# MAPieschl/PointCloudProcessing

Measured on AMD Instinct MI355X. Metric: points/sec PointNet fwd+bwd N=1024 B=32 at 1/2/4/8 MI355X vs CPU ref, higher is better.
Workload: dtype bf16; 1 GPU; PointNet-cls training step (fwd + losses + bwd + grad all-reduce + Adam), N=1024 points, batch 32 per GPU, profile classification_pretrain, 23 classes / 12 parts, random-init weights; global_batch=32, points_per_cloud=1024, parallelism=dp1, launch=hipgraph

## Files before the change

### pointcloudprocessing_amd/csrc/pn_gemm.hip

```cpp
#include <vector>
#include "pn_common.h"
#include "pn_dense_wgrad.h"
#include "pn_gemm_core.h"
#include "pn_internal.h"
#include "pn_slab_reduce.h"

namespace pn {

template <int BM, int BN, int NS, bool B2>
__global__ __launch_bounds__(256) void wgrad_batch_kernel(const WgradBatch wb) {
  __shared__ __attribute__((aligned(16))) unsigned char lds_raw[GemmLds<BM, BN, NS>::BYTES];
  wgrad_batch_tile<BM, BN, NS, B2>(wb, (int)blockIdx.x, lds_raw);
}

template <int BM, int BN, int NS, bool B2>
__global__ __launch_bounds__(256) void wgrad_batch_dense_kernel(const WgradBatch wb, int n_w, const DenseWgradBatch db) {
  __shared__ __attribute__((aligned(16))) unsigned char lds_raw[GemmLds<BM, BN, NS>::BYTES];
  static_assert(GemmLds<BM, BN, NS>::BYTES >= 16 * 32 * 4, "the dense riders' LDS tile fits");
  if ((int)blockIdx.x >= n_w) {
    dense_wgrad_batch_body(db, (int)blockIdx.x - n_w, reinterpret_cast<float(*)[32]>(lds_raw));
    return;
  }
  wgrad_batch_tile<BM, BN, NS, B2>(wb, (int)blockIdx.x, lds_raw);
}

struct WgLds {
  static constexpr int PITCH = Geo<64>::PITCH;
  static constexpr int W = 2 * 128 * PITCH, A = W + 64 * PITCH, RED_BYTES = (A + 128 * PITCH) * 2, BYTES = RED_BYTES + 4 * 64 * 4;
  static_assert(BYTES <= 65536, "the fused weight-gradient tile's LDS exceeds the static __shared__ limit");
};
template <int BM, int BN, int NS, int MODE, bool A2, int EPI, bool ADD, bool MASK, bool AH, bool S16, bool W16 = false, bool WG = false>
__device__ __forceinline__ void rows_tile_t(const GemmArgs& g, const int bx, const int by, unsigned char* lds_raw, const WgArgs* wa = nullptr) {
  constexpr int BK = (NS == 3) ? 32 : 64;
  constexpr int PITCH = Geo<BK>::PITCH;
  constexpr int MT = BM / 64, NT = BN / 64;
  constexpr int WTM = BM / 2, WTN = BN / 2;
  constexpr int TILE_A = BM * PITCH, TILE_B = BN * PITCH;
  static_assert(!WG || (BM == 128 && BN == 64 && NS == 1 && MODE == MODE_BWD && EPI == EPI_STORE && AH && S16), "the fused weight-gradient tile");
  __bf16* Ahi = reinterpret_cast<__bf16*>(lds_raw);
  __bf16* Bhi = Ahi + (WG ? WgLds::W : TILE_A);
  __bf16* Alo = (NS == 3) ? (Bhi + TILE_B) : Ahi;
  __bf16* Blo = (NS == 3) ? (Alo + TILE_A) : Bhi;

  const int tid = threadIdx.x, lane = tid & 63, wave = tid >> 6;
  const int wm = wave >> 1, wn = wave & 1;
  const int wrow0 = wm * WTM, wcol0 = wn * WTN;

  f32x16 acc[MT][NT];
#pragma unroll
  for (int m = 0; m < MT; ++m)
#pragma unroll
    for (int n = 0; n < NT; ++n)
#pragma unroll
      for (int e = 0; e < 16; ++e) acc[m][n][e] = 0.f;

  const int cloud = bx / g.tiles_per_cloud, tin = bx - cloud * g.tiles_per_cloud;

  const int row_in_cloud0 = tin * BM;
  const int nrows = min(BM, g.N - row_in_cloud0);
  const long long row0 = (long long)cloud * g.N + row_in_cloud0;
  const int col0 = by * BN;
  const long long wbase = (long long)cloud * g.w_cloud_stride;
  pn_operand wop;
  wop.s1 = g.w; wop.s2 = nullptr; wop.ca = nullptr; wop.cb = nullptr; wop.cc = nullptr;
  wop.lo = -INFINITY; wop.h16 = 0;
  wop.ld = (MODE == MODE_FWD) ? g.C : g.K;

  NatStage<BM, BK, A2, AH> sa;
  TrnStage<BN, BK, false, false> sbT;
  NatStage<BN, BK, false, false> sbN;
  CopyStage<BN, BK> sbC;
  auto issue_chunk = [&](int k0) {
    if (!(g.dbg & 4)) sa.issue(g.a, row0 * g.a.ld, nrows, k0, tid);
    if constexpr (W16) {
      sbC.issue(g.w16, (long long)col0 * g.K, g.K, g.C - col0, k0, tid);
    } else if (MODE == MODE_FWD) {
      if (!(g.dbg & 8)) sbT.issue(wop, wbase + (long long)k0 * g.C + col0, BK, g.C - col0, tid);
    } else {
      sbN.issue(wop, wbase + (long long)col0 * g.K, g.C - col0, k0, tid);
    }
  };
  NatStage<BM, BK, false, true> swg;
  if constexpr (WG) swg.issue(wa->a, row0 * wa->a.ld, nrows, 0, tid);
  if (g.K > 0) issue_chunk(0);
  for (int k0 = 0; k0 < g.K; k0 += BK) {
    sa.pin();
    if constexpr (WG) {
      Ahi = reinterpret_cast<__bf16*>(lds_raw) + (k0 / BK) * TILE_A;
      Alo = Ahi;
    }
    sa.template finish<NS>(Ahi, Alo, g.a, nrows, k0, tid);
    if constexpr (W16) {
      sbC.pin();
      sbC.finish(Bhi, g.C - col0, tid);
    } else if (MODE == MODE_FWD) {
      sbT.pin();
      sbT.template finish<NS>(Bhi, Blo, wop, BK, g.C - col0, 0, tid);
    } else {
      sbN.pin();
      sbN.template finish<NS>(Bhi, Blo, wop, g.C - col0, k0, tid);
    }
    __syncthreads();
    if (k0 + BK < g.K) issue_chunk(k0 + BK);
    mma_chunk<MT, NT, BK, NS>(acc, Ahi, Alo, Bhi, Blo, wrow0, wcol0, lane);
    __syncthreads();
  }
  if constexpr (WG) {
    swg.pin();
    swg.template finish<1>(reinterpret_cast<__bf16*>(lds_raw) + WgLds::A, reinterpret_cast<__bf16*>(lds_raw) + WgLds::A, wa->a, nrows, 0, tid);
  }

  const int r = lane & 31, h = lane >> 5;
  const bool full = (nrows == BM) && (col0 + BN <= g.C);
  float* red = reinterpret_cast<float*>(lds_raw + (WG ? WgLds::RED_BYTES : 0));

  if (EPI == EPI_STORE) {
    float s1[NT], s2[NT];
#pragma unroll
    for (int n = 0; n < NT; ++n) {
      const int jl = wcol0 + n * 32 + r, j = col0 + jl;
      const bool jv = j < g.C;
      float bias = 0.f, msc = 0.f, msh = 0.f;
      if (jv && g.cloud_bias) bias = g.cloud_bias[(long long)cloud * g.cloud_bias_stride + j];
      if (jv && g.zmask) { msc = g.msc[j]; msh = g.msh[j]; }
      float a1 = 0.f, a2 = 0.f;
#pragma unroll
      for (int m = 0; m < MT; ++m) {
        const int il0 = wrow0 + m * 32 + 4 * h;
        if (full) {
          if (g.out && !(g.dbg & 1)) epi_store_block<true, ADD, MASK, true, S16>(acc[m][n], g, row0, il0, nrows, j, jv, bias, msc, msh, a1, a2);
          else epi_store_block<true, ADD, MASK, false, S16>(acc[m][n], g, row0, il0, nrows, j, jv, bias, msc, msh, a1, a2);
        } else {
          if (g.out) epi_store_block<false, ADD, MASK, true, S16>(acc[m][n], g, row0, il0, nrows, j, jv, bias, msc, msh, a1, a2);
          else epi_store_block<false, ADD, MASK, false, S16>(acc[m][n], g, row0, il0, nrows, j, jv, bias, msc, msh, a1, a2);
        }
      }
      s1[n] = a1 + __shfl_xor(a1, 32, 64);
      s2[n] = a2 + __shfl_xor(a2, 32, 64);
    }
    if (g.stat_partials && !(g.dbg & 2)) {
      if (h == 0) {
#pragma unroll
        for (int n = 0; n < NT; ++n) {
          const int jl = wcol0 + n * 32 + r;
          red[(wm * 2 + 0) * BN + jl] = s1[n];
          red[(wm * 2 + 1) * BN + jl] = s2[n];
        }
      }
      __syncthreads();
      if (tid < BN && col0 + tid < g.C) {
        float* p = g.stat_partials + (long long)bx * 2 * g.C + col0 + tid;
        p[0] = red[0 * BN + tid] + red[2 * BN + tid];
        p[g.C] = red[1 * BN + tid] + red[3 * BN + tid];
      }
    }
    if constexpr (WG) {
      __syncthreads();
      const __bf16* img = reinterpret_cast<const __bf16*>(lds_raw);
// ... 67 lines not shown
  __shared__ __attribute__((aligned(16))) unsigned char lds_raw[LDS_BYTES];
  if constexpr (MODE == MODE_WGRAD) {
    wgrad_tile<BM, BN, NS, A2, B2>(g, blockIdx.x, blockIdx.y, blockIdx.z, lds_raw);
  } else {
    int bx = blockIdx.x, by = 0;
    const int ncol = g.ncol;
    if (ncol > 1) {
      const int lin = blockIdx.x, nrow = (int)gridDim.x / ncol, full = (nrow / 8) * 8 * ncol;
      if (lin < full) {
        const int grp = lin / (8 * ncol), r = lin - grp * 8 * ncol;
        by = r >> 3;
        bx = grp * 8 + (r & 7);
      } else {
        const int l2 = lin - full, rem = nrow - (nrow / 8) * 8;
        bx = (nrow / 8) * 8 + l2 % rem;
        by = l2 / rem;
      }
    }
    if (g.a.h16) {
      if constexpr (NS == 1 && EPI == EPI_STORE) {
        if (g.w16) {
          if (g.store16) rows_tile_t<BM, BN, NS, MODE, A2, EPI, ADD, MASK, true, true, true>(g, bx, by, lds_raw);
          else rows_tile_t<BM, BN, NS, MODE, A2, EPI, ADD, MASK, true, false, true>(g, bx, by, lds_raw);
          return;
        }
      }
      if (EPI == EPI_STORE && g.store16) rows_tile_t<BM, BN, NS, MODE, A2, EPI, ADD, MASK, true, EPI == EPI_STORE>(g, bx, by, lds_raw);
      else rows_tile_t<BM, BN, NS, MODE, A2, EPI, ADD, MASK, true, false>(g, bx, by, lds_raw);
    } else {
      if (EPI == EPI_STORE && g.store16) rows_tile_t<BM, BN, NS, MODE, A2, EPI, ADD, MASK, false, EPI == EPI_STORE>(g, bx, by, lds_raw);
      else rows_tile_t<BM, BN, NS, MODE, A2, EPI, ADD, MASK, false, false>(g, bx, by, lds_raw);
    }
  }
}

template <bool ADD, bool MASK>
__global__ __launch_bounds__(256) void gemm_bwd_wgrad_kernel(const GemmArgs g, const WgArgs wa) {
  __shared__ __attribute__((aligned(16))) unsigned char lds_raw[WgLds::BYTES];
  if (g.w16) rows_tile_t<128, 64, 1, MODE_BWD, true, EPI_STORE, ADD, MASK, true, true, true, true>(g, (int)blockIdx.x, 0, lds_raw, &wa);
  else rows_tile_t<128, 64, 1, MODE_BWD, true, EPI_STORE, ADD, MASK, true, true, false, true>(g, (int)blockIdx.x, 0, lds_raw, &wa);
}

template <bool AH, bool S16>
__global__ __launch_bounds__(256) void gemm_bwd_reduce_kernel(const GemmArgs g, int n_gemm, const float* __restrict__ slabs, int per_group,
                                                              long long elems, float* __restrict__ red_out, int nb_per_group) {
  constexpr int LDS_BYTES = (128 + 64) * Geo<64>::PITCH * 2;
  static_assert(LDS_BYTES >= 8 * 32 * 4, "the riders' LDS tile fits");
  __shared__ __attribute__((aligned(16))) unsigned char lds_raw[LDS_BYTES];
  if ((int)blockIdx.x >= n_gemm) {
    const int bx = (int)blockIdx.x - n_gemm;
    slab_reduce_block(slabs, per_group, elems, red_out, bx % nb_per_group, bx / nb_per_group, reinterpret_cast<float(*)[32]>(lds_raw));
    return;
  }
  rows_tile_t<128, 64, 1, MODE_BWD, false, EPI_STORE, false, false, AH, S16>(g, (int)blockIdx.x, 0, lds_raw);
}

template <int BM, int BN, int NS, int MODE, bool A2, bool B2, int EPI, bool ADD = false, bool MASK = false>
static int launch(const GemmArgs& g, dim3 grid, hipStream_t st) {
  hipLaunchKernelGGL((gemm_kernel<BM, BN, NS, MODE, A2, B2, EPI, ADD, MASK>), grid, dim3(256), 0, st, g);
  PN_CHECK_LAUNCH();
  return PN_OK;
}

static bool aligned16(const void* p) { return (reinterpret_cast<uintptr_t>(p) & 15) == 0; }

static int check_operand(const pn_operand* o, const char* name) {
  PN_CHECK_ARG(o && o->s1, "%s: null operand", name);
  PN_CHECK_ARG(aligned16(o->s1) && (!o->s2 || aligned16(o->s2)), "%s: s1/s2 must be 16-byte aligned", name);
  PN_CHECK_ARG((!o->ca || aligned16(o->ca)) && (!o->cb || aligned16(o->cb)) && (!o->cc || aligned16(o->cc)),
               "%s: coefficient vectors must be 16-byte aligned", name);
  PN_CHECK_ARG(o->ld > 0 && o->ld % 4 == 0, "%s: ld must be a positive multiple of 4", name);
  PN_CHECK_ARG(o->h16 == 0 || (o->h16 == 1 && o->ld % 8 == 0), "%s: h16 must be 0 or 1, and 16-bit rows need ld %% 8 == 0", name);
  return PN_OK;
}

template <int MODE, bool A2, int EPI, bool ADD = false, bool MASK = false>
static int dispatch_rows(const GemmArgs& g_in, int prec, hipStream_t st) {
  GemmArgs g = g_in;
  const bool wide = g.C % 128 == 0;
  if (EPI == EPI_MAX) {
    g.ncol = cdiv(g.C, 128);
    dim3 grid(g.B * g.tiles_per_cloud * g.ncol);
    if (prec == PN_PREC_BF16X3) return launch<128, 128, 3, MODE, A2, false, EPI>(g, grid, st);
    return launch<128, 128, 1, MODE, A2, false, EPI>(g, grid, st);
  }
  const bool few = (long long)g.B * g.tiles_per_cloud * (g.C / 128) < 64;
  if (wide && !few) {
    g.ncol = g.C / 128;
    dim3 grid(g.B * g.tiles_per_cloud * g.ncol);
    if (prec == PN_PREC_BF16X3) return launch<128, 128, 3, MODE, A2, false, EPI, ADD, MASK>(g, grid, st);
    return launch<128, 128, 1, MODE, A2, false, EPI, ADD, MASK>(g, grid, st);
  }
  g.ncol = cdiv(g.C, 64);
  dim3 grid(g.B * g.tiles_per_cloud * g.ncol);
  if (prec == PN_PREC_BF16X3) return launch<128, 64, 3, MODE, A2, false, EPI, ADD, MASK>(g, grid, st);
  return launch<128, 64, 1, MODE, A2, false, EPI, ADD, MASK>(g, grid, st);
}

template <bool A2>
static int dispatch_bwd(const GemmArgs& g, int prec, hipStream_t st) {
  const bool ha = g.addend != nullptr, hm = g.zmask != nullptr;
  if (ha && hm) return dispatch_rows<MODE_BWD, A2, EPI_STORE, true, true>(g, prec, st);
  if (ha) return dispatch_rows<MODE_BWD, A2, EPI_STORE, true, false>(g, prec, st);
  if (hm) return dispatch_rows<MODE_BWD, A2, EPI_STORE, false, true>(g, prec, st);
  return dispatch_rows<MODE_BWD, A2, EPI_STORE, false, false>(g, prec, st);
}

int conv_fwd(const pn_operand* x, const float* w, long long wcs, int B, int N, int K, int C, const float* cloud_bias,
             float* z, float* stat_partials, int prec, hipStream_t st, const void* w16) {
  PN_TRY(check_operand(x, "pn_conv_fwd.x"));
  PN_CHECK_ARG(!x->s2, "pn_conv_fwd: the forward operand has no second source");
  PN_CHECK_ARG(B > 0 && N > 0, "pn_conv_fwd: B and N must be positive (B=%d N=%d)", B, N);
  PN_CHECK_ARG(K >= 64 && K % 64 == 0, "pn_conv_fwd: K must be a multiple of 64 (K=%d)", K);
  PN_CHECK_ARG(C >= 64 && C % 64 == 0, "pn_conv_fwd: C must be a multiple of 64 (C=%d)", C);
  PN_CHECK_ARG(x->ld >= K, "pn_conv_fwd: x.ld < K");
  PN_CHECK_ARG(w && aligned16(w), "pn_conv_fwd: w null or unaligned");
  const int store16 = (prec & PN_STORE_BF16) ? 1 : 0;
  prec &= ~PN_STORE_BF16;
  PN_CHECK_ARG(prec == PN_PREC_BF16 || prec == PN_PREC_BF16X3, "pn_conv_fwd: bad prec %d", prec);
  GemmArgs g;
  memset(&g, 0, sizeof(g));
  g.store16 = store16;
  g.a = *x; g.w = w; g.w_cloud_stride = wcs; g.B = B; g.N = N; g.K = K; g.C = C;
  g.tiles_per_cloud = cdiv(N, 128);
  g.out = z; g.cloud_bias = cloud_bias; g.cloud_bias_stride = C; g.stat_partials = stat_partials;
  if (w16 && wcs == 0 && prec == PN_PREC_BF16 && x->h16 && (reinterpret_cast<uintptr_t>(w16) & 15) == 0 && K % 8 == 0)
    g.w16 = reinterpret_cast<const unsigned short*>(w16);
  static const int dbg = getenv("PN_GEMM_DBG") ? atoi(getenv("PN_GEMM_DBG")) : 0;
  g.dbg = dbg;
  return dispatch_rows<MODE_FWD, false, EPI_STORE>(g, prec, st);
}

int conv_fwd_max(const pn_operand* x, const float* w, int B, int N, int K, int C, const float* sgn, float* pmax, int* pidx,
                 float* stat_partials, int prec, hipStream_t st) {
  PN_TRY(check_operand(x, "pn_conv_fwd_max.x"));
  PN_CHECK_ARG(!x->s2, "pn_conv_fwd_max: the forward operand has no second source");
  PN_CHECK_ARG(B > 0 && N > 0, "pn_conv_fwd_max: B and N must be positive");
  PN_CHECK_ARG(K >= 64 && K % 64 == 0, "pn_conv_fwd_max: K must be a multiple of 64 (K=%d)", K);
  PN_CHECK_ARG(C >= 128 && C % 128 == 0, "pn_conv_fwd_max: C must be a multiple of 128 (C=%d)", C);
  PN_CHECK_ARG(x->ld >= K, "pn_conv_fwd_max: x.ld < K");
  PN_CHECK_ARG(w && aligned16(w) && sgn && pmax && pidx, "pn_conv_fwd_max: null pointer");
  PN_CHECK_ARG(prec == PN_PREC_BF16 || prec == PN_PREC_BF16X3, "pn_conv_fwd_max: bad prec %d", prec);
  GemmArgs g;
  memset(&g, 0, sizeof(g));
  g.a = *x; g.w = w; g.B = B; g.N = N; g.K = K; g.C = C;
  g.tiles_per_cloud = cdiv(N, 128);
  g.sgn = sgn; g.pmax = pmax; g.pidx = pidx; g.stat_partials = stat_partials;
  return dispatch_rows<MODE_FWD, false, EPI_MAX>(g, prec, st);
}

int conv_bwd_data(const pn_operand* dz, const float* w, long long wcs, int B, int N, int K, int C, const float* addend,
                  const float* zmask, const float* msc, const float* msh, float* out, float* stat_partials, int prec,
                  hipStream_t st, const void* w16, const float* col_bias, const WgradFuse* wf) {
  PN_TRY(check_operand(dz, "pn_conv_bwd_data.dz"));
  PN_CHECK_ARG(B > 0 && N > 0, "pn_conv_bwd_data: B and N must be positive");
  PN_CHECK_ARG(K >= 64 && K % 64 == 0, "pn_conv_bwd_data: K must be a multiple of 64 (K=%d)", K);
  PN_CHECK_ARG(C >= 64 && C % 64 == 0, "pn_conv_bwd_data: C must be a multiple of 64 (C=%d)", C);
  PN_CHECK_ARG(dz->ld >= K, "pn_conv_bwd_data: dz.ld < K");
  PN_CHECK_ARG(w && aligned16(w), "pn_conv_bwd_data: w null or unaligned");
  PN_CHECK_ARG(!zmask || (msc && msh), "pn_conv_bwd_data: zmask needs msc and msh");
  const int store16 = (prec & PN_STORE_BF16) ? 1 : 0;
  prec &= ~PN_STORE_BF16;
  PN_CHECK_ARG(prec == PN_PREC_BF16 || prec == PN_PREC_BF16X3, "pn_conv_bwd_data: bad prec %d", prec);
  GemmArgs g;
  memset(&g, 0, sizeof(g));
  g.store16 = store16;
  g.a = *dz; g.w = w; g.w_cloud_stride = wcs; g.B = B; g.N = N; g.K = K; g.C = C;
  g.tiles_per_cloud = cdiv(N, 128);
  g.out = out; g.addend = addend; g.zmask = zmask; g.msc = msc; g.msh = msh; g.stat_partials = stat_partials;
  g.cloud_bias = col_bias; g.cloud_bias_stride = 0;
  if (w16 && wcs == 0 && prec == PN_PREC_BF16 && dz->h16 && (reinterpret_cast<uintptr_t>(w16) & 15) == 0 && K % 8 == 0)
    g.w16 = reinterpret_cast<const unsigned short*>(w16);
  if (wf) {
    PN_TRY(check_operand(&wf->a, "pn_conv_bwd_data_wgrad.a"));
    PN_CHECK_ARG(prec == PN_PREC_BF16 && store16 && dz->h16 && dz->s2, "pn_conv_bwd_data_wgrad: bf16 operands, bf16 storage and a two-source dz");
    PN_CHECK_ARG(C == 64 && (K == 64 || K == 128), "pn_conv_bwd_data_wgrad: C must be 64 and K 64 or 128 (C=%d K=%d)", C, K);
    PN_CHECK_ARG(wf->Ci == C && wf->a.h16 && !wf->a.s2 && wf->a.ld >= wf->Ci, "pn_conv_bwd_data_wgrad: operand a must be a 64-channel bf16 single-source operand");
    PN_CHECK_ARG(wf->slab_rows == 64 || wf->slab_rows == 128, "pn_conv_bwd_data_wgrad: slab_rows must be 64 or 128 (%d)", wf->slab_rows);
    PN_CHECK_ARG(wf->slabs != nullptr, "pn_conv_bwd_data_wgrad: null slabs");
    const WgArgs wa{wf->a, wf->slabs, wf->slab_rows};
    g.ncol = 1;
    const dim3 grid(B * g.tiles_per_cloud);
    const bool ha = addend != nullptr, hm = zmask != nullptr;
    if (ha && hm) hipLaunchKernelGGL((gemm_bwd_wgrad_kernel<true, true>), grid, dim3(256), 0, st, g, wa);
    else if (ha) hipLaunchKernelGGL((gemm_bwd_wgrad_kernel<true, false>), grid, dim3(256), 0, st, g, wa);
    else if (hm) hipLaunchKernelGGL((gemm_bwd_wgrad_kernel<false, true>), grid, dim3(256), 0, st, g, wa);
    else hipLaunchKernelGGL((gemm_bwd_wgrad_kernel<false, false>), grid, dim3(256), 0, st, g, wa);
    PN_CHECK_LAUNCH();
    return PN_OK;
  }
  if (dz->s2) return dispatch_bwd<true>(g, prec, st);
  return dispatch_bwd<false>(g, prec, st);
}

int conv_bwd_data_reduce(const pn_operand* dz, const float* w, long long wcs, int B, int N, int K, int C, float* out, int prec, hipStream_t st,
                         const float* slabs, int n_slabs, int per_group, long long elems, float* red_out, bool* rode) {
  *rode = false;
  PN_TRY(check_operand(dz, "pn_conv_bwd_data.dz"));
  PN_CHECK_ARG(B > 0 && N > 0 && w && aligned16(w) && out && dz->ld >= K, "conv_bwd_data_reduce: bad arguments");
  PN_CHECK_ARG(slabs && red_out && n_slabs > 0 && per_group > 0 && n_slabs % per_group == 0 && elems > 0, "conv_bwd_data_reduce: bad sizes");
  const int store16 = (prec & PN_STORE_BF16) ? 1 : 0;
  prec &= ~PN_STORE_BF16;
  const long long nb = cdivll(elems, 32), riders = nb * (n_slabs / per_group), n_gemm = (long long)B * cdiv(N, 128);
  if (prec != PN_PREC_BF16 || dz->s2 || C != 64 || K < 64 || K % 64 != 0 || (dz->h16 != 0) != (store16 != 0) || n_gemm + riders >= (1ll << 30))
    return PN_OK;
  GemmArgs g;
  memset(&g, 0, sizeof(g));
  g.store16 = store16;
  g.a = *dz; g.w = w; g.w_cloud_stride = wcs; g.B = B; g.N = N; g.K = K; g.C = C;
  g.tiles_per_cloud = cdiv(N, 128);
  g.out = out; g.ncol = 1;
  const dim3 grid((unsigned)(n_gemm + riders));
  if (store16)
    hipLaunchKernelGGL((gemm_bwd_reduce_kernel<true, true>), grid, dim3(256), 0, st, g, (int)n_gemm, slabs, per_group, elems, red_out, (int)nb);
  else
    hipLaunchKernelGGL((gemm_bwd_reduce_kernel<false, false>), grid, dim3(256), 0, st, g, (int)n_gemm, slabs, per_group, elems, red_out, (int)nb);
  PN_CHECK_LAUNCH();
  *rode = true;
  return PN_OK;
}

template <int BM, int BN>
static int dispatch_wgrad(const GemmArgs& g, bool b2, int prec, dim3 grid, hipStream_t st) {
  if (prec == PN_PREC_BF16X3) {
    if (b2) return launch<BM, BN, 3, MODE_WGRAD, false, true, EPI_SLAB>(g, grid, st);
// ... 108 lines not shown
```

### pointcloudprocessing_amd/csrc/pn_gemm_core.h

```cpp
#pragma once
#include "pn_common.h"
#include "pn_internal.h"

namespace pn {

typedef __attribute__((ext_vector_type(8))) __bf16 bf16x8;
typedef __attribute__((ext_vector_type(16))) float f32x16;

enum { MODE_FWD = 0, MODE_BWD = 1, MODE_WGRAD = 2 };
enum { EPI_STORE = 0, EPI_MAX = 1, EPI_SLAB = 2 };

struct GemmArgs {
  pn_operand a;
  pn_operand b;
  const float* w;
  const unsigned short* w16;
  long long w_cloud_stride;
  int B, N;
  int K;
  int C;
  int Ci;
  int tiles_per_cloud;
  float* out;
  const float* cloud_bias;
  long long cloud_bias_stride;
  const float* addend;
  const float* zmask;
  const float* msc;
  const float* msh;
  float* stat_partials;
  const float* sgn;
  float* pmax;
  int* pidx;
  int store16;
  int ncol;
  int colsum;
  int dbg;
};
struct WgArgs {
  pn_operand a;
  float* slabs;
  int rows;
};

template <int BK>
struct Geo {
  static constexpr int PITCH = BK + 8;
};

__device__ __forceinline__ void cvt_store8(__bf16* hi, __bf16* lo, const float (&v)[8], bool split) {
  bf16x8 h;
#pragma unroll
  for (int e = 0; e < 8; ++e) h[e] = (__bf16)v[e];
  *reinterpret_cast<bf16x8*>(hi) = h;
  if (split) {
    bf16x8 l;
#pragma unroll
    for (int e = 0; e < 8; ++e) l[e] = (__bf16)(v[e] - (float)h[e]);
    *reinterpret_cast<bf16x8*>(lo) = l;
  }
}


template <int TR, int BK, bool HAS2, bool H16>
struct NatStage {
  static constexpr int CH = BK / 8;
  static constexpr int RP = 256 / CH;
  static constexpr int P = TR / RP;
  static constexpr int Q = H16 ? 1 : 2;
  float4 x[P][Q];
  float4 y[HAS2 ? P : 1][Q];

  __device__ __forceinline__ void issue(const pn_operand& op, long long base, int nvalid_rows, int k0, int tid) {
    const int ch = tid % CH, rin = tid / CH;
    const int k = k0 + ch * 8;
#pragma unroll
    for (int p = 0; p < P; ++p) {
      const int r = p * RP + rin;
      const long long rr = (r < nvalid_rows) ? r : (nvalid_rows - 1);
      if constexpr (H16) {
        x[p][0] = __builtin_bit_cast(float4, act_load8_raw(op.s1, base + rr * op.ld + k));
        if (HAS2) y[p][0] = __builtin_bit_cast(float4, act_load8_raw(op.s2, base + rr * op.ld + k));
      } else {
        const float* s = op.s1 + base + rr * op.ld + k;
        x[p][0] = *reinterpret_cast<const float4*>(s);
        x[p][1] = *reinterpret_cast<const float4*>(s + 4);
        if (HAS2) {
          const float* s2 = op.s2 + base + rr * op.ld + k;
          y[p][0] = *reinterpret_cast<const float4*>(s2);
          y[p][1] = *reinterpret_cast<const float4*>(s2 + 4);
        }
      }
    }
  }
  __device__ __forceinline__ void pin() {
#pragma unroll
    for (int p = 0; p < P; ++p)
#pragma unroll
      for (int q = 0; q < Q; ++q) {
        asm volatile("" : "+v"(x[p][q].x), "+v"(x[p][q].y), "+v"(x[p][q].z), "+v"(x[p][q].w));
        if (HAS2) asm volatile("" : "+v"(y[p][q].x), "+v"(y[p][q].y), "+v"(y[p][q].z), "+v"(y[p][q].w));
      }
  }
  template <int NS>
  __device__ __forceinline__ void finish(__bf16* __restrict__ Thi, __bf16* __restrict__ Tlo, const pn_operand& op,
                                         int nvalid_rows, int k0, int tid) {
    constexpr int PITCH = Geo<BK>::PITCH;
    const int ch = tid % CH, rin = tid / CH;
    const int k = k0 + ch * 8;
    float ca[8], cb[8], cc[8];
#pragma unroll
    for (int e = 0; e < 8; ++e) { ca[e] = 1.f; cb[e] = 0.f; cc[e] = 0.f; }
    if (op.ca) {
      const float4 t0 = *reinterpret_cast<const float4*>(op.ca + k), t1 = *reinterpret_cast<const float4*>(op.ca + k + 4);
      ca[0] = t0.x; ca[1] = t0.y; ca[2] = t0.z; ca[3] = t0.w; ca[4] = t1.x; ca[5] = t1.y; ca[6] = t1.z; ca[7] = t1.w;
    }
    if (HAS2 && op.cb) {
      const float4 t0 = *reinterpret_cast<const float4*>(op.cb + k), t1 = *reinterpret_cast<const float4*>(op.cb + k + 4);
      cb[0] = t0.x; cb[1] = t0.y; cb[2] = t0.z; cb[3] = t0.w; cb[4] = t1.x; cb[5] = t1.y; cb[6] = t1.z; cb[7] = t1.w;
    }
    if (op.cc) {
      const float4 t0 = *reinterpret_cast<const float4*>(op.cc + k), t1 = *reinterpret_cast<const float4*>(op.cc + k + 4);
      cc[0] = t0.x; cc[1] = t0.y; cc[2] = t0.z; cc[3] = t0.w; cc[4] = t1.x; cc[5] = t1.y; cc[6] = t1.z; cc[7] = t1.w;
    }
    const float lo = op.lo;
#pragma unroll
    for (int p = 0; p < P; ++p) {
      const int r = p * RP + rin;
      const bool rv = r < nvalid_rows;
      float v[8], w[8];
      if constexpr (H16) {
        bf16x8_unpack(__builtin_bit_cast(uint4, x[p][0]), v);
        if (HAS2) bf16x8_unpack(__builtin_bit_cast(uint4, y[p][0]), w);
      } else {
        v[0] = x[p][0].x; v[1] = x[p][0].y; v[2] = x[p][0].z; v[3] = x[p][0].w;
        v[4] = x[p][Q - 1].x; v[5] = x[p][Q - 1].y; v[6] = x[p][Q - 1].z; v[7] = x[p][Q - 1].w;
        if (HAS2) {
          w[0] = y[p][0].x; w[1] = y[p][0].y; w[2] = y[p][0].z; w[3] = y[p][0].w;
          w[4] = y[p][Q - 1].x; w[5] = y[p][Q - 1].y; w[6] = y[p][Q - 1].z; w[7] = y[p][Q - 1].w;
        }
      }
#pragma unroll
      for (int e = 0; e < 8; ++e) {
        float t = fmaf(ca[e], v[e], cc[e]);
        if (HAS2) t = fmaf(cb[e], w[e], t);
        v[e] = rv ? clamp_lo(t, lo) : 0.f;
      }
      cvt_store8(Thi + r * PITCH + ch * 8, Tlo + r * PITCH + ch * 8, v, NS == 3);
    }
  }
};

template <int TR, int BK, bool HAS2, bool H16>
struct TrnStage {
  static constexpr int KG = BK / 8;
  static constexpr int TRL = H16 ? TR / 2 : TR;
  static constexpr int TPG = 256 / TRL;
  static constexpr int P = (KG + TPG - 1) / TPG;
  static_assert(KG % TPG == 0 || TPG % KG == 0, "tile geometry");
  float x[P][8];
  float y[HAS2 ? P : 1][8];

  __device__ __forceinline__ void issue(const pn_operand& op, long long base, int nvalid_k, int nvalid_r, int tid) {
    const int rl = tid % TRL, kgin = tid / TRL;
    if constexpr (H16) {
      const int rc = (2 * rl < nvalid_r) ? 2 * rl : ((nvalid_r - 1) & ~1);
      const unsigned* p1 = reinterpret_cast<const unsigned*>(reinterpret_cast<const unsigned short*>(op.s1) + base + rc);
      const unsigned* p2 = HAS2 ? reinterpret_cast<const unsigned*>(reinterpret_cast<const unsigned short*>(op.s2) + base + rc) : nullptr;
      const long long ld2 = op.ld / 2;
#pragma unroll
      for (int p = 0; p < P; ++p) {
        const int kg = p * TPG + kgin;
#pragma unroll
        for (int e = 0; e < 8; ++e) {
          const int k = kg * 8 + e;
          const long long kk = (k < nvalid_k) ? k : (nvalid_k - 1);
          x[p][e] = __builtin_bit_cast(float, p1[kk * ld2]);
          if (HAS2) y[p][e] = __builtin_bit_cast(float, p2[kk * ld2]);
        }
      }
    } else {
      const int rc = (rl < nvalid_r) ? rl : (nvalid_r - 1);
      const float* p1 = op.s1 + base + rc;
      const float* p2 = HAS2 ? (op.s2 + base + rc) : nullptr;
#pragma unroll
      for (int p = 0; p < P; ++p) {
        const int kg = p * TPG + kgin;
#pragma unroll
        for (int e = 0; e < 8; ++e) {
          const int k = kg * 8 + e;
          const long long kk = (k < nvalid_k) ? k : (nvalid_k - 1);
          x[p][e] = p1[kk * op.ld];
          if (HAS2) y[p][e] = p2[kk * op.ld];
        }
      }
    }
  }
  __device__ __forceinline__ void pin() {
#pragma unroll
    for (int p = 0; p < P; ++p)
#pragma unroll
      for (int e = 0; e < 8; ++e) {
        asm volatile("" : "+v"(x[p][e]));
        if (HAS2) asm volatile("" : "+v"(y[p][e]));
      }
  }
  template <int NS>
  __device__ __forceinline__ float2 finish(__bf16* __restrict__ Thi, __bf16* __restrict__ Tlo, const pn_operand& op,
                                           int nvalid_k, int nvalid_r, int coef0, int tid, bool want_sum = false) {
    constexpr int PITCH = Geo<BK>::PITCH;
    constexpr int NH = H16 ? 2 : 1;
    float csum[2] = {0.f, 0.f};
    const int rl = tid % TRL, kgin = tid / TRL;
    const float lo = op.lo;
#pragma unroll
    for (int hf = 0; hf < NH; ++hf) {
      const int r = H16 ? 2 * rl + hf : rl;
      const bool rv = r < nvalid_r;
      const int rc = rv ? r : (nvalid_r - 1);
      float ca = 1.f, cb = 0.f, cc = 0.f;
      if (op.ca) ca = op.ca[coef0 + rc];
      if (HAS2 && op.cb) cb = op.cb[coef0 + rc];
      if (op.cc) cc = op.cc[coef0 + rc];
#pragma unroll
      for (int p = 0; p < P; ++p) {
        const int kg = p * TPG + kgin;
        if (KG < TPG && kg >= KG) continue;
        float v[8];
#pragma unroll
        for (int e = 0; e < 8; ++e) {
          const int k = kg * 8 + e;
          float xs, ys = 0.f;
          if constexpr (H16) {
            const unsigned ux = __builtin_bit_cast(unsigned, x[p][e]);
            xs = hf ? __builtin_bit_cast(float, ux & 0xffff0000u) : __builtin_bit_cast(float, ux << 16);
            if (HAS2) {
              const unsigned uy = __builtin_bit_cast(unsigned, y[p][e]);
              ys = hf ? __builtin_bit_cast(float, uy & 0xffff0000u) : __builtin_bit_cast(float, uy << 16);
            }
          } else {
            xs = x[p][e];
            if (HAS2) ys = y[p][e];
          }
          float t = fmaf(ca, xs, cc);
          if (HAS2) t = fmaf(cb, ys, t);
          v[e] = (rv && k < nvalid_k) ? clamp_lo(t, lo) : 0.f;
        }
        if (want_sum) csum[hf] += ((v[0] + v[1]) + (v[2] + v[3])) + ((v[4] + v[5]) + (v[6] + v[7]));
        cvt_store8(Thi + r * PITCH + kg * 8, Tlo + r * PITCH + kg * 8, v, NS == 3);
      }
    }
    return make_float2(csum[0], csum[1]);
  }
};

template <int TR, int BK>
struct CopyStage {
  static constexpr int CH = BK / 8;
  static constexpr int RP = 256 / CH;
  static constexpr int P = TR / RP;
  uint4 x[P];
  __device__ __forceinline__ void issue(const unsigned short* __restrict__ w, long long base, long long ld, int nvalid_rows, int k0, int tid) {
    const int ch = tid % CH, rin = tid / CH;
#pragma unroll
    for (int p = 0; p < P; ++p) {
      const int r = p * RP + rin;
      const long long rr = (r < nvalid_rows) ? r : (nvalid_rows - 1);
      x[p] = *reinterpret_cast<const uint4*>(w + base + rr * ld + k0 + ch * 8);
    }
  }
  __device__ __forceinline__ void pin() {
#pragma unroll
    for (int p = 0; p < P; ++p) asm volatile("" : "+v"(x[p].x), "+v"(x[p].y), "+v"(x[p].z), "+v"(x[p].w));
  }
  __device__ __forceinline__ void finish(__bf16* __restrict__ Thi, int nvalid_rows, int tid) {
    constexpr int PITCH = Geo<BK>::PITCH;
// ... 62 lines not shown
#pragma unroll
  for (int e = 0; e < 16; ++e) {
    const int il = il0 + (e & 3) + 8 * (e >> 2);
    const bool ok = FULL || (il < nrows && jv);
    float v = acc[e] + bias;
    if (HAS_ADD) v += ad[e];
    float w2 = v;
    if (HAS_MASK) {
      v = (fmaf(msc, zm[e], msh) > 0.f) ? v : 0.f;
      w2 = zm[e];
    }
    if (!FULL) v = ok ? v : 0.f;
    if (HAS_OUT) {
      if (FULL || ok) act_st<S16>(g.out, (row0 + il) * g.C + j, v);
    }
    a1 += v;
    a2 = fmaf(v, w2, a2);
  }
}

template <int BM, int BN, int NS, bool A2, bool B2, bool AH, bool BH>
__device__ __forceinline__ void wgrad_tile_t(const GemmArgs& g, const int bx, const int by, const int bz, unsigned char* lds_raw) {
  constexpr int BK = (NS == 3) ? 32 : 64;
  constexpr int PITCH = Geo<BK>::PITCH;
  constexpr int MT = BM / 64, NT = BN / 64;
  constexpr int WTM = BM / 2, WTN = BN / 2;
  constexpr int TILE_A = BM * PITCH, TILE_B = BN * PITCH;
  __bf16* Ahi = reinterpret_cast<__bf16*>(lds_raw);
  __bf16* Bhi = Ahi + TILE_A;
  __bf16* Alo = (NS == 3) ? (Bhi + TILE_B) : Ahi;
  __bf16* Blo = (NS == 3) ? (Alo + TILE_A) : Bhi;
  const int tid = threadIdx.x, lane = tid & 63, wave = tid >> 6;
  const int wm = wave >> 1, wn = wave & 1;
  const int wrow0 = wm * WTM, wcol0 = wn * WTN;
  f32x16 acc[MT][NT];
#pragma unroll
  for (int m = 0; m < MT; ++m)
#pragma unroll
    for (int n = 0; n < NT; ++n)
#pragma unroll
      for (int e = 0; e < 16; ++e) acc[m][n][e] = 0.f;
  const int cloud = bx / g.tiles_per_cloud, tin = bx - cloud * g.tiles_per_cloud;
  const int i0 = by * BM, j0 = bz * BN;
  const bool want_cs = g.colsum != 0 && bz == 0;
  float cs = 0.f, cs2 = 0.f;
  const int rbeg = tin * g.K;
  const int rend = min(g.N, rbeg + g.K);
  TrnStage<BM, BK, A2, AH> sa;
  TrnStage<BN, BK, B2, BH> sb;
  const bool same = (BM == BN) && !A2 && !B2 && (AH == BH) && i0 == j0 && g.Ci == g.C && g.a.s1 == g.b.s1 && g.a.ld == g.b.ld &&
                    g.a.ca == g.b.ca && g.a.cc == g.b.cc && g.a.lo == g.b.lo;
  const __bf16* Bh = same ? Ahi : Bhi;
  const __bf16* Bl = same ? Alo : Blo;
  if (rbeg < rend) {
    const long long rowbase = (long long)cloud * g.N + rbeg;
    const int nk = min(BK, rend - rbeg);
    sa.issue(g.a, rowbase * g.a.ld + i0, nk, g.Ci - i0, tid);
    if (!same) sb.issue(g.b, rowbase * g.b.ld + j0, nk, g.C - j0, tid);
  }
  for (int r0 = rbeg; r0 < rend; r0 += BK) {
    const int nk = min(BK, rend - r0);
    sa.pin();
    const float2 csp = sa.template finish<NS>(Ahi, Alo, g.a, nk, g.Ci - i0, i0, tid, want_cs);
    cs += csp.x; cs2 += csp.y;
    if (!same) {
      sb.pin();
      sb.template finish<NS>(Bhi, Blo, g.b, nk, g.C - j0, j0, tid);
    }
    __syncthreads();
    if (r0 + BK < rend) {
      const long long rowbase = (long long)cloud * g.N + r0 + BK;
      const int nk2 = min(BK, rend - (r0 + BK));
      sa.issue(g.a, rowbase * g.a.ld + i0, nk2, g.Ci - i0, tid);
      if (!same) sb.issue(g.b, rowbase * g.b.ld + j0, nk2, g.C - j0, tid);
    }
    mma_chunk<MT, NT, BK, NS>(acc, Ahi, Alo, Bh, Bl, wrow0, wcol0, lane);
    __syncthreads();
  }
  const long long slab_stride = (long long)g.Ci * g.C + (g.colsum ? g.Ci : 0);
  float* slab = g.out + (long long)bx * slab_stride;
  if (want_cs) {
    constexpr int TPGA = 256 / BM;
    float* red = reinterpret_cast<float*>(lds_raw);
    if constexpr (AH) {
      constexpr int BM2 = BM / 2;
      red[(tid / BM2) * BM + 2 * (tid % BM2)] = cs;
      red[(tid / BM2) * BM + 2 * (tid % BM2) + 1] = cs2;
    } else {
      red[(tid / BM) * BM + (tid % BM)] = cs;
    }
    __syncthreads();
    if (tid < BM && i0 + tid < g.Ci) {
      float t = red[tid];
      constexpr int PARTS = AH ? 2 * TPGA : TPGA;
#pragma unroll
      for (int q = 1; q < PARTS; ++q) t += red[q * BM + tid];
      slab[(long long)g.Ci * g.C + i0 + tid] = t;
    }
  }
  const int r = lane & 31, h = lane >> 5;
#pragma unroll
  for (int m = 0; m < MT; ++m)
#pragma unroll
    for (int n = 0; n < NT; ++n) {
      const int j = j0 + wcol0 + n * 32 + r;
#pragma unroll
      for (int e = 0; e < 16; ++e) {
        const int i = i0 + wrow0 + m * 32 + (e & 3) + 8 * (e >> 2) + 4 * h;
        if (i < g.Ci && j < g.C) slab[(long long)i * g.C + j] = acc[m][n][e];
      }
    }
}

typedef __attribute__((ext_vector_type(4))) short s16x4;
template <int PITCH>
__device__ __forceinline__ bf16x8 col_frag(const __bf16* img, int row0, int col0, int lane) {
  const int r = lane & 31, h = lane >> 5;
  const int i = lane & 15, q = i >> 2, p = i & 3;
  const __bf16* a0 = img + (row0 + 8 * h + q) * PITCH + col0 + (r & 16) + 4 * p;
  typedef __attribute__((address_space(3))) s16x4 lds_s16x4;
  const s16x4 lo = __builtin_amdgcn_ds_read_tr16_b64_v4i16((lds_s16x4*)(a0));
  const s16x4 hi = __builtin_amdgcn_ds_read_tr16_b64_v4i16((lds_s16x4*)(a0 + 4 * PITCH));
  typedef __attribute__((ext_vector_type(8))) short s16x8;
  const s16x8 v = __builtin_shufflevector(lo, hi, 0, 1, 2, 3, 4, 5, 6, 7);
  return __builtin_bit_cast(bf16x8, v);
}

template <int PITCH, int NJ>
// ... 99 lines not shown
```

Before: 47.00 million points/s.

## Prefetch per-channel coefficients with operand loads and double-stage two-chunk GEMM tiles

Coefficient vectors (ca/cb/cc) used when staging operands into LDS are now loaded in the issue phase alongside the operand prefetch, or once up front for the transposed stager, instead of at finish time. This hides their global-load latency behind the MMA of the previous chunk. For bf16 weight-copy tiles with K equal to two chunks, both chunks are issued before the first is staged, overlapping the loads more. The changes add register pressure from the extra prefetched registers, and a debug flag can now null the coefficient and epilogue inputs.

```diff
diff --git a/pointcloudprocessing_amd/csrc/pn_gemm.hip b/pointcloudprocessing_amd/csrc/pn_gemm.hip
--- a/pointcloudprocessing_amd/csrc/pn_gemm.hip
+++ b/pointcloudprocessing_amd/csrc/pn_gemm.hip
@@ -1,3 +1,4 @@
+#include <type_traits>
 #include <vector>
 #include "pn_common.h"
 #include "pn_dense_wgrad.h"
@@ -29,7 +30,8 @@
   static constexpr int W = 2 * 128 * PITCH, A = W + 64 * PITCH, RED_BYTES = (A + 128 * PITCH) * 2, BYTES = RED_BYTES + 4 * 64 * 4;
   static_assert(BYTES <= 65536, "the fused weight-gradient tile's LDS exceeds the static __shared__ limit");
 };
-template <int BM, int BN, int NS, int MODE, bool A2, int EPI, bool ADD, bool MASK, bool AH, bool S16, bool W16 = false, bool WG = false>
+template <int BM, int BN, int NS, int MODE, bool A2, int EPI, bool ADD, bool MASK, bool AH, bool S16, bool W16 = false, bool WG = false,
+          bool CPRE = true>
 __device__ __forceinline__ void rows_tile_t(const GemmArgs& g, const int bx, const int by, unsigned char* lds_raw, const WgArgs* wa = nullptr) {
   constexpr int BK = (NS == 3) ? 32 : 64;
   constexpr int PITCH = Geo<BK>::PITCH;
@@ -66,44 +68,75 @@
   wop.lo = -INFINITY; wop.h16 = 0;
   wop.ld = (MODE == MODE_FWD) ? g.C : g.K;
 
-  NatStage<BM, BK, A2, AH> sa;
-  TrnStage<BN, BK, false, false> sbT;
-  NatStage<BN, BK, false, false> sbN;
-  CopyStage<BN, BK> sbC;
-  auto issue_chunk = [&](int k0) {
-    if (!(g.dbg & 4)) sa.issue(g.a, row0 * g.a.ld, nrows, k0, tid);
+  constexpr bool ASIS = MODE == MODE_BWD && ADD && MASK && BN == 128 && !WG;
+  struct Stagers {
+    NatStage<BM, BK, A2, AH, (CPRE && !ASIS) ? 2 : 1> a;
+    std::conditional_t<W16, CopyStage<BN, BK>,
+                       std::conditional_t<MODE == MODE_FWD, TrnStage<BN, BK, false, false, false>, NatStage<BN, BK, false, false, 0>>> b;
+  };
+  auto issue_chunk = [&](Stagers& s, int k0) {
+    if (!(g.dbg & 4)) s.a.issue(g.a, row0 * g.a.ld, nrows, k0, tid);
     if constexpr (W16) {
-      sbC.issue(g.w16, (long long)col0 * g.K, g.K, g.C - col0, k0, tid);
-    } else if (MODE == MODE_FWD) {
-      if (!(g.dbg & 8)) sbT.issue(wop, wbase + (long long)k0 * g.C + col0, BK, g.C - col0, tid);
+      s.b.issue(g.w16, (long long)col0 * g.K, g.K, g.C - col0, k0, tid);
+    } else if constexpr (MODE == MODE_FWD) {
+      if (!(g.dbg & 8)) s.b.issue(wop, wbase + (long long)k0 * g.C + col0, BK, g.C - col0, tid);
     } else {
-      sbN.issue(wop, wbase + (long long)col0 * g.K, g.C - col0, k0, tid);
-    }
+      s.b.issue(wop, wbase + (long long)col0 * g.K, g.C - col0, k0, tid);
+    }
+  };
+  auto stage_chunk = [&](Stagers& s, int k0) {
+    s.a.pin();
+    if constexpr (WG) {
+      Ahi = reinterpret_cast<__bf16*>(lds_raw) + (k0 / BK) * TILE_A;
+      Alo = Ahi;
+    }
+    s.a.template finish<NS>(Ahi, Alo, g.a, nrows, k0, tid);
+    s.b.pin();
+    if constexpr (W16) s.b.finish(Bhi, g.C - col0, tid);
+    else if constexpr (MODE == MODE_FWD) s.b.template finish<NS>(Bhi, Blo, wop, BK, g.C - col0, 0, tid);
+    else s.b.template finish<NS>(Bhi, Blo, wop, g.C - col0, k0, tid);
+    __syncthreads();
+  };
+  auto mma = [&]() {
+    mma_chunk<MT, NT, BK, NS>(acc, Ahi, Alo, Bhi, Blo, wrow0, wcol0, lane);
+    __syncthreads();
   };
   NatStage<BM, BK, false, true> swg;
   if constexpr (WG) swg.issue(wa->a, row0 * wa->a.ld, nrows, 0, tid);
-  if (g.K > 0) issue_chunk(0);
-  for (int k0 = 0; k0 < g.K; k0 += BK) {
-    sa.pin();
-    if constexpr (WG) {
-      Ahi = reinterpret_cast<__bf16*>(lds_raw) + (k0 / BK) * TILE_A;
-      Alo = Ahi;
-    }
-    sa.template finish<NS>(Ahi, Alo, g.a, nrows, k0, tid);
-    if constexpr (W16) {
-      sbC.pin();
-      sbC.finish(Bhi, g.C - col0, tid);
-    } else if (MODE == MODE_FWD) {
-      sbT.pin();
-      sbT.template finish<NS>(Bhi, Blo, wop, BK, g.C - col0, 0, tid);
-    } else {
-      sbN.pin();
-      sbN.template finish<NS>(Bhi, Blo, wop, g.C - col0, k0, tid);
-    }
-    __syncthreads();
-    if (k0 + BK < g.K) issue_chunk(k0 + BK);
-    mma_chunk<MT, NT, BK, NS>(acc, Ahi, Alo, Bhi, Blo, wrow0, wcol0, lane);
-    __syncthreads();
+  bool staged = false;
+  if constexpr (AH && W16 && (MODE == MODE_FWD || WG)) {
+    if (g.K == 2 * BK) {
+      Stagers s0, s1;
+      issue_chunk(s0, 0);
+      issue_chunk(s1, BK);
+      stage_chunk(s0, 0);
+      mma();
+      stage_chunk(s1, BK);
+      mma();
+      staged = true;
+    }
+  }
+  if constexpr (ASIS) {
+    Stagers s;
+    issue_chunk(s, 0);
+    for (int k0 = 0; k0 < g.K; k0 += BK) {
+      stage_chunk(s, k0);
+      if (k0 + BK < g.K) issue_chunk(s, k0 + BK);
+      mma();
+    }
+    staged = true;
+  }
+  if (!staged) {
+    Stagers s;
+    issue_chunk(s, 0);
+    int k0 = 0;
+    for (; k0 + BK < g.K; k0 += BK) {
+      stage_chunk(s, k0);
+      issue_chunk(s, k0 + BK);
+      mma();
+    }
+    stage_chunk(s, k0);
+    mma();
   }
   if constexpr (WG) {
     swg.pin();
@@ -277,7 +310,7 @@
     slab_reduce_block(slabs, per_group, elems, red_out, bx % nb_per_group, bx / nb_per_group, reinterpret_cast<float(*)[32]>(lds_raw));
     return;
   }
-  rows_tile_t<128, 64, 1, MODE_BWD, false, EPI_STORE, false, false, AH, S16>(g, (int)blockIdx.x, 0, lds_raw);
+  rows_tile_t<128, 64, 1, MODE_BWD, false, EPI_STORE, false, false, AH, S16, false, false, false>(g, (int)blockIdx.x, 0, lds_raw);
 }
 
 template <int BM, int BN, int NS, int MODE, bool A2, bool B2, int EPI, bool ADD = false, bool MASK = false>
@@ -352,7 +385,8 @@
   if (w16 && wcs == 0 && prec == PN_PREC_BF16 && x->h16 && (reinterpret_cast<uintptr_t>(w16) & 15) == 0 && K % 8 == 0)
     g.w16 = reinterpret_cast<const unsigned short*>(w16);
   static const int dbg = getenv("PN_GEMM_DBG") ? atoi(getenv("PN_GEMM_DBG")) : 0;
-  g.dbg = dbg;
+  g.dbg = dbg & 15;
+  if (dbg & 16) { g.a.ca = nullptr; g.a.cb = nullptr; g.a.cc = nullptr; }
   return dispatch_rows<MODE_FWD, false, EPI_STORE>(g, prec, st);
 }
 
@@ -396,6 +430,12 @@
   g.cloud_bias = col_bias; g.cloud_bias_stride = 0;
   if (w16 && wcs == 0 && prec == PN_PREC_BF16 && dz->h16 && (reinterpret_cast<uintptr_t>(w16) & 15) == 0 && K % 8 == 0)
     g.w16 = reinterpret_cast<const unsigned short*>(w16);
+  static const int dbg = getenv("PN_GEMM_DBG") ? atoi(getenv("PN_GEMM_DBG")) : 0;
+  if (dbg & 16) {
+    g.a.ca = nullptr; g.a.cb = nullptr; g.a.cc = nullptr;
+    g.addend = nullptr; g.zmask = nullptr; g.msc = nullptr; g.msh = nullptr;
+    addend = nullptr; zmask = nullptr;
+  }
   if (wf) {
     PN_TRY(check_operand(&wf->a, "pn_conv_bwd_data_wgrad.a"));
     PN_CHECK_ARG(prec == PN_PREC_BF16 && store16 && dz->h16 && dz->s2, "pn_conv_bwd_data_wgrad: bf16 operands, bf16 storage and a two-source dz");
diff --git a/pointcloudprocessing_amd/csrc/pn_gemm_core.h b/pointcloudprocessing_amd/csrc/pn_gemm_core.h
--- a/pointcloudprocessing_amd/csrc/pn_gemm_core.h
+++ b/pointcloudprocessing_amd/csrc/pn_gemm_core.h
@@ -62,7 +62,7 @@
 }
 
 
-template <int TR, int BK, bool HAS2, bool H16>
+template <int TR, int BK, bool HAS2, bool H16, int COEF = 2>
 struct NatStage {
   static constexpr int CH = BK / 8;
   static constexpr int RP = 256 / CH;
@@ -70,10 +70,23 @@
   static constexpr int Q = H16 ? 1 : 2;
   float4 x[P][Q];
   float4 y[HAS2 ? P : 1][Q];
+  static constexpr bool PREF = COEF == 2 && H16;
+  float4 ka[PREF ? 2 : 1], kb[(PREF && HAS2) ? 2 : 1], kc[PREF ? 2 : 1];
 
   __device__ __forceinline__ void issue(const pn_operand& op, long long base, int nvalid_rows, int k0, int tid) {
     const int ch = tid % CH, rin = tid / CH;
     const int k = k0 + ch * 8;
+    if constexpr (PREF) {
+      const float4* spare = reinterpret_cast<const float4*>(op.s1);
+      const float4* pa = op.ca ? reinterpret_cast<const float4*>(op.ca + k) : spare;
+      const float4* pc = op.cc ? reinterpret_cast<const float4*>(op.cc + k) : spare;
+      ka[0] = pa[0]; ka[1] = pa[1];
+      if constexpr (HAS2) {
+        const float4* pb = op.cb ? reinterpret_cast<const float4*>(op.cb + k) : spare;
+        kb[0] = pb[0]; kb[1] = pb[1];
+      }
+      kc[0] = pc[0]; kc[1] = pc[1];
+    }
 #pragma unroll
     for (int p = 0; p < P; ++p) {
       const int r = p * RP + rin;
@@ -101,6 +114,14 @@
         asm volatile("" : "+v"(x[p][q].x), "+v"(x[p][q].y), "+v"(x[p][q].z), "+v"(x[p][q].w));
         if (HAS2) asm volatile("" : "+v"(y[p][q].x), "+v"(y[p][q].y), "+v"(y[p][q].z), "+v"(y[p][q].w));
       }
+    if constexpr (PREF) {
+#pragma unroll
+      for (int q = 0; q < 2; ++q) {
+        asm volatile("" : "+v"(ka[q].x), "+v"(ka[q].y), "+v"(ka[q].z), "+v"(ka[q].w));
+        if constexpr (HAS2) asm volatile("" : "+v"(kb[q].x), "+v"(kb[q].y), "+v"(kb[q].z), "+v"(kb[q].w));
+        asm volatile("" : "+v"(kc[q].x), "+v"(kc[q].y), "+v"(kc[q].z), "+v"(kc[q].w));
+      }
+    }
   }
   template <int NS>
   __device__ __forceinline__ void finish(__bf16* __restrict__ Thi, __bf16* __restrict__ Tlo, const pn_operand& op,
@@ -111,18 +132,33 @@
     float ca[8], cb[8], cc[8];
 #pragma unroll
     for (int e = 0; e < 8; ++e) { ca[e] = 1.f; cb[e] = 0.f; cc[e] = 0.f; }
-    if (op.ca) {
-      const float4 t0 = *reinterpret_cast<const float4*>(op.ca + k), t1 = *reinterpret_cast<const float4*>(op.ca + k + 4);
-      ca[0] = t0.x; ca[1] = t0.y; ca[2] = t0.z; ca[3] = t0.w; ca[4] = t1.x; ca[5] = t1.y; ca[6] = t1.z; ca[7] = t1.w;
-    }
-    if (HAS2 && op.cb) {
-      const float4 t0 = *reinterpret_cast<const float4*>(op.cb + k), t1 = *reinterpret_cast<const float4*>(op.cb + k + 4);
-      cb[0] = t0.x; cb[1] = t0.y; cb[2] = t0.z; cb[3] = t0.w; cb[4] = t1.x; cb[5] = t1.y; cb[6] = t1.z; cb[7] = t1.w;
-    }
-    if (op.cc) {
-      const float4 t0 = *reinterpret_cast<const float4*>(op.cc + k), t1 = *reinterpret_cast<const float4*>(op.cc + k + 4);
-      cc[0] = t0.x; cc[1] = t0.y; cc[2] = t0.z; cc[3] = t0.w; cc[4] = t1.x; cc[5] = t1.y; cc[6] = t1.z; cc[7] = t1.w;
-    }
+    if constexpr (PREF) {
+      if (op.ca) {
+        ca[0] = ka[0].x; ca[1] = ka[0].y; ca[2] = ka[0].z; ca[3] = ka[0].w; ca[4] = ka[1].x; ca[5] = ka[1].y; ca[6] = ka[1].z; ca[7] = ka[1].w;
+      }
+      if constexpr (HAS2) {
+        if (op.cb) {
+          cb[0] = kb[0].x; cb[1] = kb[0].y; cb[2] = kb[0].z; cb[3] = kb[0].w; cb[4] = kb[1].x; cb[5] = kb[1].y; cb[6] = kb[1].z; cb[7] = kb[1].w;
+        }
+      }
+      if (op.cc) {
+        cc[0] = kc[0].x; cc[1] = kc[0].y; cc[2] = kc[0].z; cc[3] = kc[0].w; cc[4] = kc[1].x; cc[5] = kc[1].y; cc[6] = kc[1].z; cc[7] = kc[1].w;
+      }
+    } else if constexpr (COEF != 0) {
+      if (op.ca) {
+        const float4 t0 = *reinterpret_cast<const float4*>(op.ca + k), t1 = *reinterpret_cast<const float4*>(op.ca + k + 4);
+        ca[0] = t0.x; ca[1] = t0.y; ca[2] = t0.z; ca[3] = t0.w; ca[4] = t1.x; ca[5] = t1.y; ca[6] = t1.z; ca[7] = t1.w;
+      }
+      if (HAS2 && op.cb) {
+        const float4 t0 = *reinterpret_cast<const float4*>(op.cb + k), t1 = *reinterpret_cast<const float4*>(op.cb + k + 4);
+        cb[0] = t0.x; cb[1] = t0.y; cb[2] = t0.z; cb[3] = t0.w; cb[4] = t1.x; cb[5] = t1.y; cb[6] = t1.z; cb[7] = t1.w;
+      }
+      if (op.cc) {
+        const float4 t0 = *reinterpret_cast<const float4*>(op.cc + k), t1 = *reinterpret_cast<const float4*>(op.cc + k + 4);
+        cc[0] = t0.x; cc[1] = t0.y; cc[2] = t0.z; cc[3] = t0.w; cc[4] = t1.x; cc[5] = t1.y; cc[6] = t1.z; cc[7] = t1.w;
+      }
+    }
+    (void)k;
     const float lo = op.lo;
 #pragma unroll
     for (int p = 0; p < P; ++p) {
@@ -151,7 +187,7 @@
   }
 };
 
-template <int TR, int BK, bool HAS2, bool H16>
+template <int TR, int BK, bool HAS2, bool H16, bool COEF = true>
 struct TrnStage {
   static constexpr int KG = BK / 8;
   static constexpr int TRL = H16 ? TR / 2 : TR;
@@ -160,7 +196,22 @@
   static_assert(KG % TPG == 0 || TPG % KG == 0, "tile geometry");
   float x[P][8];
   float y[HAS2 ? P : 1][8];
-
+  static constexpr int NH = H16 ? 2 : 1;
+  float ka[NH], kb[NH], kc[NH];
+
+  __device__ __forceinline__ void coefs(const pn_operand& op, int nvalid_r, int coef0, int tid) {
+    const int rl = tid % TRL;
+    const float* spare = reinterpret_cast<const float*>(op.s1);
+#pragma unroll
+    for (int hf = 0; hf < NH; ++hf) {
+      const int r = H16 ? 2 * rl + hf : rl;
+      const int rc = (r < nvalid_r) ? r : (nvalid_r - 1);
+      ka[hf] = *(op.ca ? op.ca + coef0 + rc : spare);
+      if constexpr (HAS2) kb[hf] = *(op.cb ? op.cb + coef0 + rc : spare);
+      else kb[hf] = 0.f;
+      kc[hf] = *(op.cc ? op.cc + coef0 + rc : spare);
+    }
+  }
   __device__ __forceinline__ void issue(const pn_operand& op, long long base, int nvalid_k, int nvalid_r, int tid) {
     const int rl = tid % TRL, kgin = tid / TRL;
     if constexpr (H16) {
@@ -204,12 +255,15 @@
         asm volatile("" : "+v"(x[p][e]));
         if (HAS2) asm volatile("" : "+v"(y[p][e]));
       }
+    if constexpr (COEF) {
+#pragma unroll
+      for (int hf = 0; hf < NH; ++hf) asm volatile("" : "+v"(ka[hf]), "+v"(kb[hf]), "+v"(kc[hf]));
+    }
   }
   template <int NS>
   __device__ __forceinline__ float2 finish(__bf16* __restrict__ Thi, __bf16* __restrict__ Tlo, const pn_operand& op,
                                            int nvalid_k, int nvalid_r, int coef0, int tid, bool want_sum = false) {
     constexpr int PITCH = Geo<BK>::PITCH;
-    constexpr int NH = H16 ? 2 : 1;
     float csum[2] = {0.f, 0.f};
     const int rl = tid % TRL, kgin = tid / TRL;
     const float lo = op.lo;
@@ -217,11 +271,12 @@
     for (int hf = 0; hf < NH; ++hf) {
       const int r = H16 ? 2 * rl + hf : rl;
       const bool rv = r < nvalid_r;
-      const int rc = rv ? r : (nvalid_r - 1);
       float ca = 1.f, cb = 0.f, cc = 0.f;
-      if (op.ca) ca = op.ca[coef0 + rc];
-      if (HAS2 && op.cb) cb = op.cb[coef0 + rc];
-      if (op.cc) cc = op.cc[coef0 + rc];
+      if constexpr (COEF) {
+        if (op.ca) ca = ka[hf];
+        if (HAS2 && op.cb) cb = kb[hf];
+        if (op.cc) cc = kc[hf];
+      }
 #pragma unroll
       for (int p = 0; p < P; ++p) {
         const int kg = p * TPG + kgin;
@@ -390,13 +445,13 @@
                     g.a.ca == g.b.ca && g.a.cc == g.b.cc && g.a.lo == g.b.lo;
   const __bf16* Bh = same ? Ahi : Bhi;
   const __bf16* Bl = same ? Alo : Blo;
-  if (rbeg < rend) {
-    const long long rowbase = (long long)cloud * g.N + rbeg;
-    const int nk = min(BK, rend - rbeg);
+  auto issue_chunk = [&](int r0) {
+    const long long rowbase = (long long)cloud * g.N + r0;
+    const int nk = min(BK, rend - r0);
     sa.issue(g.a, rowbase * g.a.ld + i0, nk, g.Ci - i0, tid);
     if (!same) sb.issue(g.b, rowbase * g.b.ld + j0, nk, g.C - j0, tid);
-  }
-  for (int r0 = rbeg; r0 < rend; r0 += BK) {
+  };
+  auto stage_chunk = [&](int r0) {
     const int nk = min(BK, rend - r0);
     sa.pin();
     const float2 csp = sa.template finish<NS>(Ahi, Alo, g.a, nk, g.Ci - i0, i0, tid, want_cs);
@@ -406,12 +461,19 @@
       sb.template finish<NS>(Bhi, Blo, g.b, nk, g.C - j0, j0, tid);
     }
     __syncthreads();
-    if (r0 + BK < rend) {
-      const long long rowbase = (long long)cloud * g.N + r0 + BK;
-      const int nk2 = min(BK, rend - (r0 + BK));
-      sa.issue(g.a, rowbase * g.a.ld + i0, nk2, g.Ci - i0, tid);
-      if (!same) sb.issue(g.b, rowbase * g.b.ld + j0, nk2, g.C - j0, tid);
-    }
+  };
+  if (rbeg < rend) {
+    sa.coefs(g.a, g.Ci - i0, i0, tid);
+    if (!same) sb.coefs(g.b, g.C - j0, j0, tid);
+    issue_chunk(rbeg);
+    int r0 = rbeg;
+    for (; r0 + BK < rend; r0 += BK) {
+      stage_chunk(r0);
+      issue_chunk(r0 + BK);
+      mma_chunk<MT, NT, BK, NS>(acc, Ahi, Alo, Bh, Bl, wrow0, wcol0, lane);
+      __syncthreads();
+    }
+    stage_chunk(r0);
     mma_chunk<MT, NT, BK, NS>(acc, Ahi, Alo, Bh, Bl, wrow0, wcol0, lane);
     __syncthreads();
   }
```

Result: no change. 47.41 million points/s, median of 6 (+0.9%).
